# Visual-Behavior/detr-tensorflow

Hardware: AMD Instinct MI355X
Metric: images/sec training step, DETR-R50 800x1333 bs=8/GPU (higher is better)
Workload: dtype bf16

## Files before the change

### detr-tensorflow_amd/csrc/common.h

```cpp
#pragma once
#include <hip/hip_runtime.h>
#include <stdint.h>
#include <stdio.h>
#include <stdarg.h>
#include <stdlib.h>

#include "../../include/detr_hip.h"

namespace detr {

void set_error(const char *fmt, ...);

#define DETR_REQUIRE(cond, ...)                 \
    do {                                        \
        if (!(cond)) {                          \
            ::detr::set_error(__VA_ARGS__);     \
            return -1;                          \
        }                                       \
    } while (0)

#define DETR_LAUNCH_CHECK(name)                                                         \
    do {                                                                                \
        hipError_t e__ = hipGetLastError();                                             \
        if (e__ != hipSuccess) {                                                        \
// ... 32 lines not shown
    T_DGRAD_S2_CLASSES,
    T_WGRAD_FUSED,
    T_WGRAD_FUSED_WGS,
    T_WGRAD_TILE,
    T_STEM_ROWS,
    T_ATTN_WAVES,
    T_ATTN_SPLIT,
    T_GEMM_K64,
    T_EPI_WIDE,
    T_SLAB_TS,
    T_GEMM_RING,
    T_RING_NS,
    T_RING_BN,
    T_RING_WGS,
    T_RING_ROWS,
    T_RING_WTILE,
    T_CONV_DMA,
    T_SPLIT3_T128,
    T_X3_DB,
    T_X3_T192,
    T_X3_WG_ROUNDS,
    T_X3_CONV,
    T_SPLIT3_ALL,
    T_COUNT
};
int tune(TuneKey k);

static inline bool aligned16(const void *p) { return (reinterpret_cast<uintptr_t>(p) & 15) == 0; }
static inline int cdiv(long long a, long long b) { return (int)((a + b - 1) / b); }
static inline int capped_grid(long long total, int block, int cap) {
    const long long g = (total + block - 1) / block;
    return (int)(g > cap ? cap : (g < 1 ? 1 : g));
}

__host__ __device__ __forceinline__ uint32_t mix32(uint32_t x) {
    x ^= x >> 16; x *= 0x7feb352du;
    x ^= x >> 15; x *= 0x846ca68bu;
    x ^= x >> 16;
    return x;
}
__host__ __device__ __forceinline__ uint32_t drop_key(uint32_t site, const uint32_t *step) {
    return mix32((step ? *step : 0u) + site * 0x9E3779B9u);
}
__host__ __device__ __forceinline__ uint32_t drop_hash(uint32_t key, unsigned long long pair) {
    const uint32_t key2 = key * 0x85EBCA6Bu + 0xC2B2AE35u;
    uint32_t x = (uint32_t)pair ^ key;
// ... 40 lines not shown
```

### detr-tensorflow_amd/csrc/common.hip

```cpp
#include "common.h"
#include <string.h>

namespace detr {
static thread_local char g_err[512] = "";
void set_error(const char *fmt, ...) {
    va_list ap;
    va_start(ap, fmt);
    vsnprintf(g_err, sizeof(g_err), fmt, ap);
    va_end(ap);
}
static const char *const g_tune_names[T_COUNT] = {
    "DETR_HIP_GEMM_TILE",
    "DETR_HIP_SPLIT_XCD",
    "DETR_HIP_GEMM_STREAM",
    "DETR_HIP_GEMM_GROUP",
    "DETR_HIP_STREAM_SL",
    "DETR_HIP_STREAM_NW",
    "DETR_HIP_CONV_HALO",
    "DETR_HIP_CONV_TILE",
    "DETR_HIP_DGRAD_S2_CLASSES",
    "DETR_HIP_WGRAD_FUSED",
    "DETR_HIP_WGRAD_FUSED_WGS",
    "DETR_HIP_WGRAD_TILE",
    "DETR_HIP_STEM_ROWS",
    "DETR_HIP_ATTN_WAVES",
    "DETR_HIP_ATTN_SPLIT",
    "DETR_HIP_GEMM_K64",
    "DETR_HIP_EPI_WIDE",
    "DETR_HIP_SLAB_TS",
    "DETR_HIP_GEMM_RING",
    "DETR_HIP_RING_NS",
    "DETR_HIP_RING_BN",
    "DETR_HIP_RING_WGS",
    "DETR_HIP_RING_ROWS",
    "DETR_HIP_RING_WTILE",
    "DETR_HIP_CONV_DMA",
    "DETR_HIP_SPLIT3_T128",
    "DETR_HIP_X3_DB",
    "DETR_HIP_X3_T192",
    "DETR_HIP_X3_WG_ROUNDS",
    "DETR_HIP_X3_CONV",
    "DETR_HIP_SPLIT3_ALL",
};
static int g_tune[T_COUNT];
static void load_tuning() {
    for (int i = 0; i < T_COUNT; ++i) {
        const char *v = getenv(g_tune_names[i]);
        __atomic_store_n(&g_tune[i], v ? atoi(v) : 0, __ATOMIC_RELAXED);
    }
}
static const bool g_tune_loaded = (load_tuning(), true);
int tune(TuneKey k) { return __atomic_load_n(&g_tune[k], __ATOMIC_RELAXED); }
}

extern "C" int detr_hip_reload_tuning(void) {
    detr::load_tuning();
    return 0;
}
extern "C" const char *detr_hip_last_error(void) { return detr::g_err; }
extern "C" int detr_hip_abi_version(void) { return DETR_HIP_ABI_VERSION; }
__global__ __launch_bounds__(256) void zero_fill_kernel(uint4 *__restrict__ p16, size_t n16, unsigned char *__restrict__ tail, int ntail) {
    const uint4 z = make_uint4(0u, 0u, 0u, 0u);
    for (size_t i = blockIdx.x * (size_t)blockDim.x + threadIdx.x; i < n16; i += (size_t)gridDim.x * blockDim.x) p16[i] = z;
    if (blockIdx.x == 0 && (int)threadIdx.x < ntail) tail[threadIdx.x] = 0;
}
// ... 206 lines not shown
```

### detr-tensorflow_amd/csrc/gemm_f32.hip

```cpp
#include "gemm_core.h"
#include "gemm_bf16_core.h"
#include "gemm_stream.h"

#include "gemm_kernels.h"
#include "gemm_x3.h"
#include "gemm_ring.h"

namespace detr {

struct ReduceOne {
    const float *ws; int splits; long long part_stride; int rows, cols; float *C; long long ldc;
    float alpha; const float *scale; int vec; const float *rs_ws; float *rs_out; float rs_alpha; int nblocks;
    int ts_bm, ts_bn, ts_tn;
};
struct ReduceGroupArgs { ReduceOne r[GEMM_MAX_GROUP]; };

template <int G>
__device__ __forceinline__ void splitk_reduce_body(const float *__restrict__ ws, int splits, long long part_stride,
                                                   int rows, int cols, float *__restrict__ C, long long ldc,
                                                   float alpha, const float *__restrict__ scale, int vec,
                                                   const float *__restrict__ rs_ws, float *__restrict__ rs_out,
                                                   float rs_alpha, const int bid, const int nbid,
                                                   const int ts_bm = 0, const int ts_bn = 0, const int ts_tn = 1) {
    constexpr int OUT = 256 / G;
// ... 537 lines not shown
    if (!(p.bf16c && g.a16 && g.b16 && p.ak && p.batch == 1 && p.split == 1 && !g.rowsum && !d->ln_y)) return false;
    if (!(d->K % RING_BK == 0 && d->K >= 2 * RING_BK && d->N >= 128 && d->N % 8 == 0 && d->lda % 8 == 0 && d->ldb % 8 == 0 && aligned16(d->A) &&
          aligned16(d->B))) return false;
    const bool tall = d->M >= 4096 && d->K >= 512;
    const bool dec_ffn = d->M >= 512 && d->K >= 1024;
    const bool k256 = d->K == 256 && d->N >= 1024 && (d->M >= 16384 || (d->M >= 4096 && !p.bk));
    if (mode != 1 && !(tall || dec_ffn || k256)) return false;
    return gemm_ring_plan(d->M, d->N, d->K, rp);
}

static bool gemm_ring_f32_eligible(const GemmPlan &p, RingPlan &rp) {
    const detr_gemm_desc *d = p.d;
    const GemmArgs &g = p.g;
    const int mode = tune(T_GEMM_RING);
    if (mode == 2) return false;
    if (p.bf16c || p.split3 || g.a16 || g.b16 || !p.ak || p.batch != 1 || p.split != 1 || g.rowsum || d->ln_y) return false;
    if (d->c_dtype || d->r_dtype || d->m_dtype) return false;
    if (!(d->K % 32 == 0 && d->K >= 64 && d->N >= 128 && d->lda % 4 == 0 && d->ldb % 4 == 0 && aligned16(d->A) && aligned16(d->B) &&
          (p.bk || d->N % 4 == 0))) return false;
    if (mode != 1 && !(d->M >= 16384)) return false;
    return gemm_ring_f32_plan(d->M, d->N, d->K, rp);
}

static int gemm_launch(const GemmPlan &p, hipStream_t s) {
    const GemmArgs &g = p.g;
    const detr_gemm_desc *d = p.d;
    const int batch = p.batch;
    const bool ak = p.ak, bk = p.bk;
    if (d->ln_y) return gemm_ln_launch(p, s);
    {
        RingPlan rp;
        const bool ring_first = tune(T_GEMM_STREAM) != 3 && gemm_ring_eligible(p, rp);
        if (!ring_first && gemm_stream_eligible(p)) {
            gemm_stream_launch(p, s);
            DETR_LAUNCH_CHECK("gemm (stream)");
            return 0;
        }
        if (ring_first) {
            if (gemm_ring_launch(g, bk, rp, s)) return -1;
            DETR_LAUNCH_CHECK("gemm (ring)");
            if (d->defer_out) d->defer_out->splits = 0;
            return 0;
        }
        if (gemm_ring_f32_eligible(p, rp)) {
            if (gemm_ring_f32_launch(g, bk, rp, s)) return -1;
            DETR_LAUNCH_CHECK("gemm (ring, fp32)");
            if (d->defer_out) d->defer_out->splits = 0;
            return 0;
        }
    }
    const bool ring_wgrad = p.bf16c && (p.tile == 1 || p.tile == 6 || p.tile == 7) && g.a16 && g.b16 && !ak && !bk && batch == 1 && p.split > 1 &&
                            g.slab_ts && !g.rowsum && d->M % 8 == 0 && d->N % 8 == 0 && d->lda % 8 == 0 && d->ldb % 8 == 0 && aligned16(d->A) &&
                            aligned16(d->B) && tune(T_GEMM_RING) != 2 && tune(T_GEMM_RING) != 3;
    DETR_REQUIRE(ring_wgrad || (p.tile != 6 && p.tile != 7), "gemm: the 128 x 256 / 256 x 128 tiles exist for the ring weight gradient only "
                 "(tile-ordered slabs in a workspace of detr_hip_workspace_bytes_gemm bytes are required)");
    if (ring_wgrad) {
        if (gemm_ring_wgrad_launch(g, p.ts_bm, p.ts_bn, p.split, s)) return -1;
    } else if (p.bf16c) {
        if (p.tile == 2) launch_cfg_bf16<128, 64, 2, 2>(g, batch, s, ak, bk);
        else if (p.tile == 4) launch_cfg_bf16<64, 128, 2, 2>(g, batch, s, ak, bk);
        else if (p.tile == 0) launch_cfg_bf16<64, 64, 2, 2>(g, batch, s, ak, bk, p.deep);
        else launch_cfg_bf16<128, 128, 2, 2>(g, batch, s, ak, bk, p.deep);
    } else if (p.split3 && p.tile == 8) launch_x3<192, 128>(g, batch, s, ak, bk);
    else if (p.split3 && p.tile == 1) launch_x3<128, 128>(g, batch, s, ak, bk);
    else if (p.split3 && p.tile == 2) launch_x3<128, 64>(g, batch, s, ak, bk);
    else if (p.split3) launch_x3<64, 64>(g, batch, s, ak, bk);
    else if (p.tile == 1) launch_cfg<128, 128, 2, 2>(g, batch, s, ak, bk);
    else if (p.tile == 2) launch_cfg<128, 64, 2, 2>(g, batch, s, ak, bk);
    else if (p.tile == 3) launch_cfg<128, 32, 4, 1>(g, batch, s, ak, bk);
    else if (p.tile == 4) launch_cfg<64, 256, 1, 4>(g, batch, s, ak, bk);
    else if (p.tile == 5) launch_cfg<256, 64, 4, 1>(g, batch, s, ak, bk);
    else launch_cfg<64, 64, 2, 2>(g, batch, s, ak, bk);
    DETR_LAUNCH_CHECK("gemm");
    if (p.partial && d->defer_out) {
        detr_reduce_desc *o = d->defer_out;
        o->ws = d->workspace; o->splits = p.split; o->part_stride = p.part; o->rows = d->M; o->cols = d->N;
// ... 2 lines not shown
        o->rs_out = d->rowsum_a; o->rs_alpha = d->rowsum_alpha;
        o->ts_bm = p.ts_bm; o->ts_bn = p.ts_bn; o->ts_tiles_n = p.ts_tn;
        return 0;
    }
    if (d->defer_out) d->defer_out->splits = 0;
    if (p.partial) {
        launch_splitk_reduce(d->workspace, p.split, p.part, d->M, d->N, d->C, d->ldc, p.final_e.alpha, p.final_e.scale, s,
                             d->rowsum_a ? d->workspace + (long long)p.split * p.part : nullptr, d->rowsum_a, d->rowsum_alpha,
                             p.ts_bm, p.ts_bn, p.ts_tn);
        DETR_LAUNCH_CHECK("gemm split-k reduce");
    }
    return 0;
}

extern "C" int detr_hip_gemm_family(const detr_gemm_desc *d) {
    GemmPlan p;
    if (gemm_prepare(d, p)) return -1;
    if (d->ln_y) return 4;
    RingPlan rp;
    const bool ring_first = tune(T_GEMM_STREAM) != 3 && gemm_ring_eligible(p, rp);
    if (!ring_first && gemm_stream_eligible(p)) return 1;
    if (ring_first) return 2;
    if (gemm_ring_f32_eligible(p, rp)) return 3;
    const GemmArgs &g = p.g;
    const bool ring_wgrad = p.bf16c && (p.tile == 1 || p.tile == 6 || p.tile == 7) && g.a16 && g.b16 && !p.ak && !p.bk && p.batch == 1 && p.split > 1 &&
                            g.slab_ts && !g.rowsum && d->M % 8 == 0 && d->N % 8 == 0 && d->lda % 8 == 0 && d->ldb % 8 == 0 && aligned16(d->A) &&
                            aligned16(d->B) && tune(T_GEMM_RING) != 2 && tune(T_GEMM_RING) != 3;
    return ring_wgrad ? 5 : 0;
}

extern "C" int detr_hip_gemm_f32(const detr_gemm_desc *d, void *stream) {
    GemmPlan p;
    if (gemm_prepare(d, p)) return -1;
    return gemm_launch(p, (hipStream_t)stream);
}

template <bool AK, bool BKC>
static void launch_group_f32(const GemmGroupArgs &G, dim3 grid, hipStream_t s, bool split3) {
    if (split3) hipLaunchKernelGGL((gemm_x3_group_kernel<64, 64, AK, BKC>), grid, dim3(GEMM_THREADS), 0, s, G);
    else hipLaunchKernelGGL((gemm_f32_group_kernel<64, 64, 2, 2, AK, BKC>), grid, dim3(GEMM_THREADS), 0, s, G);
}
template <bool AK, bool BKC, bool A16, bool B16>
static void launch_group_bf16(const GemmGroupArgs &G, dim3 grid, hipStream_t s) {
    hipLaunchKernelGGL((gemm_bf16c_group_kernel<64, 64, 2, 2, AK, BKC, A16, B16>), grid, dim3(GEMM_THREADS), 0, s, G);
}

extern "C" int detr_hip_gemm_group_f32(const detr_gemm_desc *descs, int32_t n, void *stream) {
    DETR_REQUIRE(descs != nullptr && n >= 1 && n <= 64, "gemm group: 1..64 descriptors");
    hipStream_t s = (hipStream_t)stream;
    int done = 0;
    while (done < n) {
        const int m = (n - done) < GEMM_MAX_GROUP ? (n - done) : GEMM_MAX_GROUP;
        GemmPlan p[GEMM_MAX_GROUP];
        for (int i = 0; i < m; ++i) {
            DETR_REQUIRE(!descs[done + i].ln_y, "gemm group: the fused LayerNorm (ln_y) exists for single launches only");
            if (gemm_prepare(descs + done + i, p[i])) return -1;
        }
        bool same = m > 1 && tune(T_GEMM_GROUP) != 2;
        for (int i = 0; i < m && same; ++i)
            same = p[i].tile == 0 && p[i].batch == 1 && p[i].bf16c == p[0].bf16c && p[i].split3 == p[0].split3 && p[i].ak == p[0].ak && p[i].bk == p[0].bk &&
                   p[i].g.a16 == p[0].g.a16 && p[i].g.b16 == p[0].g.b16 && (p[i].split == 1 || p[i].partial) &&
                   !gemm_stream_eligible(p[i]);
        if (same) { RingPlan rp; for (int i = 0; i < m && same; ++i) same = !gemm_ring_eligible(p[i], rp) && !gemm_ring_f32_eligible(p[i], rp); }
        if (!same) {
            for (int i = 0; i < m; ++i)
                if (gemm_launch(p[i], s)) return -1;
            done += m;
            continue;
        }
        GemmGroupArgs G;
        G.n = m;
        G.work_off[0] = 0;
        for (int i = 0; i < m; ++i) {
            G.g[i] = p[i].g;
            G.g[i].tiles_m = cdiv(p[i].g.M, 64);
            G.g[i].tiles_n = cdiv(p[i].g.N, 64);
            G.work_off[i + 1] = G.work_off[i] + G.g[i].tiles_m * G.g[i].tiles_n * p[i].split;
        }
        for (int i = m; i < GEMM_MAX_GROUP; ++i) { G.g[i] = G.g[0]; G.work_off[i + 1] = G.work_off[m]; }
        const dim3 grid((unsigned)G.work_off[m]);
        const bool ak = p[0].ak, bk = p[0].bk, a16 = p[0].g.a16 != 0, b16 = p[0].g.b16 != 0;
#define DETR_GROUP_BF16(A16_, B16_)                                          \
    do {                                                                     \
        if (ak && bk) launch_group_bf16<true, true, A16_, B16_>(G, grid, s);    \
        else if (ak) launch_group_bf16<true, false, A16_, B16_>(G, grid, s);    \
        else if (bk) launch_group_bf16<false, true, A16_, B16_>(G, grid, s);    \
        else launch_group_bf16<false, false, A16_, B16_>(G, grid, s);           \
    } while (0)
        if (p[0].bf16c) {
            if (a16 && b16) DETR_GROUP_BF16(true, true);
            else if (a16) DETR_GROUP_BF16(true, false);
            else if (b16) DETR_GROUP_BF16(false, true);
            else DETR_GROUP_BF16(false, false);
        } else if (ak && bk) launch_group_f32<true, true>(G, grid, s, p[0].split3);
        else if (ak) launch_group_f32<true, false>(G, grid, s, p[0].split3);
        else if (bk) launch_group_f32<false, true>(G, grid, s, p[0].split3);
        else launch_group_f32<false, false>(G, grid, s, p[0].split3);
#undef DETR_GROUP_BF16
        DETR_LAUNCH_CHECK("gemm group");
        ReduceGroupArgs R;
        int nr = 0;
        unsigned rx = 1;
        bool all_small = true, any_small = false;
        for (int i = 0; i < m; ++i) {
            const detr_gemm_desc *d = p[i].d;
            if (d->defer_out) {
                detr_reduce_desc *o = d->defer_out;
                o->splits = 0;
                if (p[i].partial) {
                    o->ws = d->workspace; o->splits = p[i].split; o->part_stride = p[i].part; o->rows = d->M; o->cols = d->N;
                    o->C = d->C; o->ldc = d->ldc; o->alpha = p[i].final_e.alpha; o->scale = p[i].final_e.scale;
                    o->rs_ws = d->rowsum_a ? d->workspace + (long long)p[i].split * p[i].part : nullptr;
// ... 77 lines not shown
```

### detr-tensorflow_amd/csrc/gemm_ring.h

```cpp
#pragma once
#include "gemm_kernels.h"

namespace detr {

typedef __attribute__((address_space(3))) void lds_void_t;
constexpr int RING_BK = 64;
constexpr int RING_THREADS = 512;
constexpr int RING_STAGE_ROW = RING_BK * 2;

struct RingArgs {
    GemmArgs g;
    int tile_rows;
    int a_rows8;
    int stage_bytes;
    int dump_off;
};

struct RingPlan {
    int tm, tn, ns;
    int tile_rows, tiles_m, tiles_n, wgs;
    int a_rows8, stage_bytes, dump_off, lds_bytes;
    double cost;
};
bool gemm_ring_plan(int M, int N, int K, RingPlan &p);
int gemm_ring_wgrad_launch(const GemmArgs &g, int bm, int bn, int split, hipStream_t s);
int gemm_ring_launch(const GemmArgs &g, bool b_kcontig, const RingPlan &p, hipStream_t s);
bool gemm_ring_f32_plan(int M, int N, int K, RingPlan &p);
int gemm_ring_f32_launch(const GemmArgs &g, bool b_kcontig, const RingPlan &p, hipStream_t s);

template <int N>
__device__ __forceinline__ void ring_wait_vmcnt() {
    static_assert(N >= 0 && N < 64, "vmcnt is a 6-bit counter");
    asm volatile("s_waitcnt vmcnt(%0)" ::"n"(N) : "memory");
}

__device__ __forceinline__ void ring_dma_piece(u32x4 rs, unsigned lds_addr, unsigned voff) {
    asm volatile("s_mov_b32 m0, %0\n\ts_nop 0\n\tbuffer_load_dwordx4 %1, %2, 0 offen lds" ::"s"(lds_addr), "v"(voff), "s"(rs) : "memory", "m0");
}
__device__ __forceinline__ u32x4 ring_rsrc(const void *base, unsigned bytes) {
    const unsigned long long b = (unsigned long long)base;
    u32x4 r;
    r[0] = (unsigned)b;
    r[1] = (unsigned)(b >> 32) & 0xFFFFu;
    r[2] = bytes;
    r[3] = 0x00020000u;
    return r;
}
__device__ __forceinline__ unsigned ring_lds_addr(char *p) {
// ... 382 lines not shown
            __builtin_amdgcn_sched_barrier(0);
            cur = (cur + 1 == NS) ? 0 : cur + 1;
            nxt = (nxt + 1 == NS) ? 0 : nxt + 1;
        }
    };
    if (nmi == TM) kloop(std::integral_constant<int, TM>{});
    else if (TM >= 2 && nmi == TM - 1) kloop(std::integral_constant<int, (TM >= 2 ? TM - 1 : 0)>{});
    else if (TM >= 3 && nmi == TM - 2) kloop(std::integral_constant<int, (TM >= 3 ? TM - 2 : 0)>{});
    else if (TM >= 4 && nmi == TM - 3) kloop(std::integral_constant<int, (TM >= 4 ? TM - 3 : 0)>{});
    else kloop(std::integral_constant<int, 0>{});
    ring_wait_vmcnt<0>();
    __syncthreads();
    epilogue<BM, BN, WGM, WGN, false>(acc, reinterpret_cast<float *>(ring_smem), g.C, g.ldc, row_end, g.N, m0, n0, wm, wn, lane, wave, g.e);
}

template <int TM, int TN, bool BKC, int NS>
__global__ __launch_bounds__(RING_THREADS) void gemm_ring_f32_kernel(RingArgs ra) {
#if defined(__HIP_DEVICE_COMPILE__)
    gemm_ring_f32_body<TM, TN, BKC, NS>(ra, xcd_remap((int)blockIdx.x, (int)gridDim.x));
#endif
}

template <int TM, int TN, int NS>
__device__ __forceinline__ void gemm_ring_wgrad_body(const RingArgs &ra) {
    constexpr int BM = 64 * TM, BN = 128 * TN, WGM = 2, WGN = 4;
    static_assert(TM % 2 == 0, "the A image is made of 128-row pieces");
    using T = TileCfg<BM, BN, WGM, WGN>;
    extern __shared__ __attribute__((aligned(1024))) char ring_smem[];
    const GemmArgs &g = ra.g;
    const int tid = threadIdx.x, lane = tid & 63;
    const int wave = __builtin_amdgcn_readfirstlane(tid >> 6);
    const int wm = wave / WGN, wn = wave % WGN;
    const int tiles = g.tiles_m * g.tiles_n;
    const int id = xcd_remap((int)blockIdx.x, (int)gridDim.x);
    const int tile = id % tiles, split = id / tiles;
    const int tn = tile % g.tiles_n, tm = tile / g.tiles_n;
    const int m0 = tm * BM, n0 = tn * BN;
    const int nkt32 = (g.K + BF_BK - 1) / BF_BK;
    const int per = (nkt32 + g.split_k - 1) / g.split_k;
    const int kbeg = split * per * BF_BK;
    const int kend = min(g.K, kbeg + per * BF_BK);
    if (kbeg >= kend) return;
    RingDmaMN<BM> la;
    RingDmaMN<BN> lb;
    la.init(g.A, g.lda, m0, g.M, kend, lane, wave);
    lb.init(g.B, g.ldb, n0, g.N, kend, lane, wave);
    f32x16 acc[TM][TN];
#pragma unroll
    for (int i = 0; i < TM; ++i)
#pragma unroll
        for (int j = 0; j < TN; ++j)
#pragma unroll
            for (int r = 0; r < 16; ++r) acc[i][j][r] = 0.0f;
    constexpr int A_BYTES = BM * RING_STAGE_ROW, STAGE = (BM + BN) * RING_STAGE_ROW, PW = TM + 2 * TN;
    const unsigned lds0 = ring_lds_addr(ring_smem);
    int atr[TM], btr[TN];
#pragma unroll
// ... 15 lines not shown
        ring_stage<TM, TM, TN, false, false>(ring_smem + cur * STAGE, ring_smem + cur * STAGE + A_BYTES, acc, 0, atr, 0, btr, xo, la, lb,
                                             kbeg + (t + NS - 1) * RING_BK, kend, lds0, nxt * STAGE, nxt * STAGE + A_BYTES, 0);
        __builtin_amdgcn_sched_barrier(0);
        cur = (cur + 1 == NS) ? 0 : cur + 1;
        nxt = (nxt + 1 == NS) ? 0 : nxt + 1;
    }
    ring_wait_vmcnt<0>();
    float4 *slab = reinterpret_cast<float4 *>(g.C + (long long)split * g.part_stride + (long long)tile * (BM * BN));
    const int w2 = 2 * wm + (wn >> 1);
#pragma unroll
    for (int mi = 0; mi < TM; ++mi)
#pragma unroll
        for (int ni = 0; ni < TN; ++ni) {
            const int blk = (w2 * TM + mi) * (2 * TN) + (wn & 1) * TN + ni;
#pragma unroll
            for (int q = 0; q < 4; ++q)
                slab[(blk * 4 + q) * 64 + lane] = make_float4(acc[mi][ni][4 * q], acc[mi][ni][4 * q + 1], acc[mi][ni][4 * q + 2], acc[mi][ni][4 * q + 3]);
        }
}

template <int TM, int TN, int NS>
__global__ __launch_bounds__(RING_THREADS) void gemm_ring_wgrad_kernel(RingArgs ra) {
#if defined(__HIP_DEVICE_COMPILE__)
    gemm_ring_wgrad_body<TM, TN, NS>(ra);
#endif
}

}
```

### detr-tensorflow_amd/csrc/gemm_ring.hip

```cpp
#include "gemm_ring.h"

namespace detr {

bool gemm_ring_plan(int M, int N, int K, RingPlan &p) {
    if (M < 1 || N < 128 || K < RING_BK || K % RING_BK != 0) return false;
    const int force_bn = tune(T_RING_BN), force_wgs = tune(T_RING_WGS), force_ns = tune(T_RING_NS), force_rows = tune(T_RING_ROWS);
    int bn = 128;
    if (force_bn == 256 && N >= 256) bn = 256;
    const int tiles_n = cdiv(N, bn);
    int rows = 176, ns = 2;
    if (cdiv(M, 176) * tiles_n < 320) {
        rows = (int)(((long long)M * tiles_n + 199) / 200);
        rows = (rows + 3) & ~3;
        if (rows > 176) rows = 176;
        ns = 3;
    }
    if (force_wgs > 0) {
        const int tm_ = force_wgs / tiles_n > 0 ? force_wgs / tiles_n : 1;
        rows = (cdiv(M, tm_) + 3) & ~3;
    }
    if (force_rows >= 8) rows = (force_rows + 3) & ~3;
    if (rows < 8) rows = 8;
    if (rows > 256) return false;
    p.tile_rows = rows;
// ... 122 lines not shown
    if (!reserved) {
        hipError_t e = hipFuncSetAttribute(reinterpret_cast<const void *>(gemm_ring_wgrad_kernel<TM, TN, NS>), hipFuncAttributeMaxDynamicSharedMemorySize, 160 * 1024);
        DETR_REQUIRE(e == hipSuccess, "gemm (ring wgrad): cannot reserve LDS: %s", hipGetErrorString(e));
        reserved = true;
    }
    hipLaunchKernelGGL((gemm_ring_wgrad_kernel<TM, TN, NS>), dim3((unsigned)wgs), dim3(RING_THREADS), (size_t)LDS, s, ra);
    return 0;
}

int gemm_ring_wgrad_launch(const GemmArgs &g, int bm, int bn, int split, hipStream_t s) {
    RingArgs ra;
    ra.g = g;
    ra.g.tiles_m = cdiv(g.M, bm);
    ra.g.tiles_n = cdiv(g.N, bn);
    ra.tile_rows = ra.a_rows8 = ra.stage_bytes = ra.dump_off = 0;
    const int wgs = ra.g.tiles_m * ra.g.tiles_n * split;
    if (bm == 128 && bn == 128) return tune(T_RING_NS) == 3 ? ring_wgrad_launch_one<2, 1, 3>(ra, wgs, s) : ring_wgrad_launch_one<2, 1, 4>(ra, wgs, s);
    if (bm == 128 && bn == 256) return ring_wgrad_launch_one<2, 2, 3>(ra, wgs, s);
    if (bm == 256 && bn == 128) return ring_wgrad_launch_one<4, 1, 3>(ra, wgs, s);
    DETR_REQUIRE(false, "gemm (ring wgrad): no instantiation for %d x %d tiles", bm, bn);
    return -1;
}

}

extern "C" int detr_hip_gemm_ring_plan(int32_t M, int32_t N, int32_t K, int32_t *out) {
    detr::RingPlan p;
    if (!detr::gemm_ring_plan(M, N, K, p)) return 0;
    if (out) {
        out[0] = p.tm; out[1] = p.tn; out[2] = p.ns; out[3] = p.tile_rows; out[4] = p.tiles_m; out[5] = p.tiles_n; out[6] = p.wgs; out[7] = p.lds_bytes;
    }
    return 1;
}
```

### detr-tensorflow_amd/detr_tf/_hip.py

```python
import ctypes
import os
from ctypes import POINTER, Structure, byref, c_float, c_int32, c_int64, c_size_t, c_void_p

import torch

_HERE = os.path.dirname(os.path.abspath(__file__))
LIB_PATH = os.environ.get("DETR_HIP_LIB") or os.path.join(os.path.dirname(_HERE), "lib", "libdetr_hip.so")

f32p = c_void_p


class ReduceDesc(Structure):
    _fields_ = [("ws", c_void_p), ("splits", c_int32), ("part_stride", c_int64), ("rows", c_int32), ("cols", c_int32),
                ("C", c_void_p), ("ldc", c_int64), ("alpha", c_float), ("scale", c_void_p),
                ("rs_ws", c_void_p), ("rs_out", c_void_p), ("rs_alpha", c_float),
                ("ts_bm", c_int32), ("ts_bn", c_int32), ("ts_tiles_n", c_int32)]


class GemmDesc(Structure):
    _fields_ = [("M", c_int32), ("N", c_int32), ("K", c_int32),
                ("A", c_void_p), ("lda", c_int64), ("a_kcontig", c_int32),
                ("B", c_void_p), ("ldb", c_int64), ("b_kcontig", c_int32),
                ("C", c_void_p), ("ldc", c_int64),
                ("batch", c_int32), ("batch_inner", c_int32),
# ... 162 lines not shown
                ("t_crowd", c_void_p), ("t_area", c_void_p), ("sM_b", c_int64), ("sizes", c_void_p),
                ("thresholds", ctypes.c_double * COCO_MAX_THR), ("area_ranges", ctypes.c_double * (2 * COCO_MAX_AREA)),
                ("rec_score", c_void_p), ("rec_class", c_void_p), ("rec_rank", c_void_p), ("rec_flags", c_void_p),
                ("npig", c_void_p), ("status", c_void_p)]


class SetLossDesc(Structure):
    _fields_ = [("levels", c_int32), ("B", c_int32), ("Q", c_int32), ("C", c_int32), ("R", c_int32),
                ("logits", c_void_p), ("sL_l", c_int64), ("sL_b", c_int64), ("sL_q", c_int64),
                ("boxes", c_void_p), ("sB_l", c_int64), ("sB_b", c_int64), ("sB_q", c_int64),
                ("t_bbox", c_void_p), ("t_class", c_void_p),
                ("background_class", c_int32)]


_SIGNATURES = {
    "detr_hip_abi_version": [],
    "detr_hip_reload_tuning": [],
    "detr_hip_struct_layout": [c_int32, POINTER(c_int32), c_int32],
    "detr_hip_memset_zero": [c_void_p, c_size_t, c_void_p],
    "detr_hip_gemm_f32": [POINTER(GemmDesc), c_void_p],
    "detr_hip_gemm_group_f32": [POINTER(GemmDesc), c_int32, c_void_p],
    "detr_hip_gemm_family": [POINTER(GemmDesc)],
    "detr_hip_gemm_ring_plan": [c_int32, c_int32, c_int32, POINTER(c_int32)],
    "detr_hip_splitk_reduce_many": [POINTER(ReduceDesc), c_int32, c_void_p],
    "detr_hip_conv3x3_f32": [POINTER(Conv3x3Desc), c_int32, c_void_p],
    "detr_hip_maxpool3x3s2_fwd_bf16": [c_void_p, c_void_p, c_void_p, c_int32, c_int32, c_int32, c_int32, c_int32, c_int32, c_void_p],
    "detr_hip_maxpool3x3s2_bwd_bf16": [c_void_p, c_void_p, c_void_p, c_void_p, c_int32, c_int32, c_int32, c_int32, c_int32, c_int32,
                                       c_void_p],
    "detr_hip_cvt_bf16": [f32p, c_void_p, c_int64, c_void_p],
    "detr_hip_scale_cols_bf16": [f32p, f32p, c_void_p, c_int64, c_int32, c_void_p],
    "detr_hip_scale_cols_bf16_group": [c_void_p, c_int32, c_void_p],
    "detr_hip_stem_conv7x7_f32": [POINTER(StemDesc), c_int32, c_void_p],
    "detr_hip_maxpool3x3s2_fwd_f32": [f32p, f32p, c_void_p, c_int32, c_int32, c_int32, c_int32, c_int32, c_int32, c_void_p],
    "detr_hip_maxpool3x3s2_bwd_f32": [f32p, c_void_p, f32p, f32p, c_int32, c_int32, c_int32, c_int32, c_int32, c_int32, c_void_p],
    "detr_hip_subsample2_fwd_f32": [f32p, f32p, c_int32, c_int32, c_int32, c_int32, c_int32, c_int32, c_void_p],
    "detr_hip_subsample2_bwd_f32": [f32p, f32p, c_int32, c_int32, c_int32, c_int32, c_int32, c_int32, c_void_p],
    "detr_hip_layernorm_fwd": [POINTER(LayerNormDesc), c_void_p],
    "detr_hip_layernorm_bwd": [POINTER(LayerNormDesc), c_void_p],
    "detr_hip_attention_fwd": [POINTER(AttnDesc), c_void_p],
    "detr_hip_attention_bwd": [POINTER(AttnDesc), c_void_p],
    "detr_hip_attention_dropmask": [POINTER(AttnDesc), c_void_p],
    "detr_hip_attention_dropmask_many": [POINTER(AttnDesc), c_int32, c_void_p],
    "detr_hip_attention_fwd_masked": [POINTER(AttnDesc), c_void_p, c_void_p],
    "detr_hip_attention_bwd_masked": [POINTER(AttnDesc), c_void_p, c_void_p],
    "detr_hip_attention_weights": [POINTER(AttnDesc), c_void_p, c_void_p, c_int64, c_void_p],
    "detr_hip_padding_mask_prepare": [c_void_p, c_int32, c_int32, c_int32, c_int32, c_int32, f32p, f32p, c_void_p, f32p, c_void_p, c_void_p],
# ... 751 lines not shown
```

### detr-tensorflow_amd/detr_tf/engine.py

```python
import math
import os
from ctypes import byref, c_float

import numpy as np
import torch

from . import _hip as hip
from .params import ParamStore, RESNET50_BLOCKS, block_names, bn_conv_pairs, stem_names

D = 256
HEADS = 8
HD = 32
FF = 2048
BN_EPS = 1e-5
KERAS_BN_EPS = 1.001e-5
LN_EPS = 1e-5
DEFER_REDUCE = os.environ.get("DETR_HIP_DEFER_REDUCE", "1") != "0"
WGRAD_STREAM = os.environ.get("DETR_HIP_WGRAD_STREAM", "1") != "0"
BWD_FUSED = os.environ.get("DETR_HIP_BWD_FUSED", "1") != "0"
DROPMASK_AHEAD = int(os.environ.get("DETR_HIP_DROPMASK_AHEAD", "2") or 0)
QK_ALPHA = float(HD) ** -0.5 * 1.4426950408889634


def mix32(x):
    x &= 0xFFFFFFFF
    x ^= x >> 16
    x = (x * 0x7FEB352D) & 0xFFFFFFFF
    x ^= x >> 15
    x = (x * 0x846CA68B) & 0xFFFFFFFF
    x ^= x >> 16
    return x


def step_seed(base_seed, step_no, rank=0):
    return mix32(mix32((base_seed + 0x9E3779B9 * step_no) & 0xFFFFFFFF) ^ ((rank * 0x85EBCA6B) & 0xFFFFFFFF))


def position_embedding_sine_host(H, W, num_pos_features=128, temperature=10000.0, eps=1e-6):
    y = (np.arange(1, H + 1, dtype=np.float32) / np.float32(H + eps) * np.float32(2 * math.pi)).astype(np.float32)
    x = (np.arange(1, W + 1, dtype=np.float32) / np.float32(W + eps) * np.float32(2 * math.pi)).astype(np.float32)
    k = np.arange(num_pos_features, dtype=np.float32)
# ... 191 lines not shown
            self._fold_table = torch.tensor(rows, dtype=torch.int64).to(self.device)
            self._fold_keep = [self.bn_scale, self._bufs]
        hip.call("detr_hip_scale_cols_bf16_group", self._fold_table.data_ptr(), self._fold_table.shape[0])

    def _scaled_kernel(self, conv_name, bn_name):
        w = self.P.views[conv_name]
        co = w.shape[-1]
        if self.compute == 1 and conv_name != f"{self._stem['conv']}/kernel":
            return self.buf(f"ws16:{conv_name}", w.shape, torch.bfloat16)
        ws = self.buf(f"ws:{conv_name}", w.shape)
        if self._stale(f"ws:{conv_name}"):
            hip.call("detr_hip_scale_cols_f32", w.data_ptr(), self.bn_scale[bn_name].data_ptr(), ws.data_ptr(),
                     w.numel() // co, co)
        return ws

    def _conv1x1_fwd(self, x, M, cin, cout, conv_name, bn_name, out, residual=None, act=1, maskbits_out=None):
        ws = self._scaled_kernel(conv_name, bn_name)
        shift = self.bn_shift[bn_name]
        ldr = cout if residual is not None else 0
        hip.gemm(M, cout, cin, x, cin, 1, ws, cout, 0, out, cout, bias=shift, residual=residual, ldr=ldr, act=act,
                 maskbits_out=maskbits_out)

    @staticmethod
    def _wgrad(M_out, N_out, K_red, A, lda, Bm, ldb, C, ldc, scale=None, alpha=1.0):
        sk = hip.pick_split_k(M_out, N_out, K_red)
        if sk > 1:
            hip.gemm(M_out, N_out, K_red, A, lda, 0, Bm, ldb, 0, C, ldc, alpha=alpha, scale=scale, split_k=sk)
        else:
            hip.gemm(M_out, N_out, K_red, A, lda, 0, Bm, ldb, 0, C, ldc, alpha=alpha, scale=scale, residual=C, ldr=ldc)

    def _colsum(self, x2d, out, alpha=1.0):
        rows, cols = x2d.shape
        n = int(hip.load().detr_hip_colsum_det_scratch_floats(rows, cols))
        scratch = self.buf(f"colsum:{rows}x{cols}", (n,))
        hip.call("detr_hip_colsum_det_f32", x2d.data_ptr(), out.data_ptr(), rows, cols, x2d.stride(0), c_float(alpha),
                 scratch.data_ptr(), n)

    def _ln_fwd(self, x, pfx, y, tag, add=None, y2=None, y16=None):
        rows = x.shape[0]
        mean = self.buf(f"{tag}:mean", (rows,))
        rstd = self.buf(f"{tag}:rstd", (rows,))
        hip.layernorm_fwd(x, self.P.views[f"{pfx}/gamma"], self.P.views[f"{pfx}/beta"], y, mean, rstd, LN_EPS, add=add, y2=y2,
                          y16=y16)

    def _ln_spec(self, rows, pfx, y, tag, add=None, y2=None, y16=None, ffn=False):
        if self.compute != 1 or ffn:
            return None
        return dict(gamma=self.P.views[f"{pfx}/gamma"], beta=self.P.views[f"{pfx}/beta"], y=y, mean=self.buf(f"{tag}:mean", (rows,)),
                    rstd=self.buf(f"{tag}:rstd", (rows,)), eps=LN_EPS, add=add, y2=y2, y16=y16)

    def _side_begin(self, on):
        self._side_on = bool(on)
# ... 687 lines not shown
            fused_ok = BWD_FUSED and self.compute == 1 and adt == torch.bfloat16 and d2 == 256 and g.is_cuda
            fuse3, fuse_down = fused_ok and d1 == 64, False
            if m["first"] and not (tfb and strided):
                idg = self.buf(f"scratch:idg:{cin}:{h}", (B, h, w, cin), adt)

                fuse_down = fused_ok and not strided and cin == 64

                def dg_down(g=g, idg=idg):
                    if strided:
                        dxs = self.buf(f"scratch:dxs:{cin}:{ho}", (B, ho, wo, cin), adt)
                        hip.gemm(M_out, cin, d2, g, d2, 1, wsd, d2, 1, dxs, cin)
                        hip.call("detr_hip_subsample2_bwd_f32", dxs.data_ptr(), idg.data_ptr(), B, h, w, cin // f32c, ho, wo)
                    elif fuse_down:
                        hip.conv1x1_bwd_fused(g.view(M_out, d2), xs.view(M_out, cin), wsd.view(cin, d2), idg.view(M_out, cin), G[f"{n['down']}/kernel"].view(cin, d2),
                                              self.buf(f"bwdfused:slabs:down:{M_out}", (hip.conv1x1_bwd_fused_scratch_floats(M_out),)),
                                              scale=self.bn_scale[n["bnd"]], use_mask=False)
                    else:
                        hip.gemm(M_out, cin, d2, g, d2, 1, wsd, d2, 1, idg, cin)
                on_side(dg_down)
                if ws_on:
                    idg_ready = torch.cuda.Event()
                    idg_ready.record(wside)

            def wg3(g=g, fuse3=fuse3, fuse_down=fuse_down):
                if not fuse3:
                    self._wgrad(d1, d2, M_out, y2, d1, g, d2, G[f"{n['conv3']}/kernel"], d2, scale=self.bn_scale[n["bn3"]])
                bias_grad(n["conv3"], n["bn3"], g, M_out, d2)
                if m["first"]:
                    if not fuse_down:
                        self._wgrad(cin, d2, M_out, xs, cin, g, d2, G[f"{n['down']}/kernel"], d2, scale=self.bn_scale[n["bnd"]])
                    bias_grad(n["down"], n["bnd"], g, M_out, d2)
            on_side(wg3)
            dz2 = self.buf(f"scratch:dz2:{d1}:{ho}{par}", (B, ho, wo, d1), adt)
            if fuse3:
                hip.conv1x1_bwd_fused(g.view(M_out, d2), y2.view(M_out, d1), ws3.view(d1, d2), dz2.view(M_out, d1), G[f"{n['conv3']}/kernel"].view(d1, d2),
                                      self.buf(f"bwdfused:slabs:{M_out}", (hip.conv1x1_bwd_fused_scratch_floats(M_out),)),
                                      scale=self.bn_scale[n["bn3"]], use_mask=True)
            else:
                hip.gemm(M_out, d1, d2, g, d2, 1, ws3, d2, 1, dz2, d1, mask=y2, ldmask=d1)

            def wg2():
                hip.conv3x3(2, y1, dz2, G[f"{n['conv2']}/kernel"], B, h1, w1, d1, ho, wo, d1, s2, scale=self.bn_scale[n["bn2"]],
                            pad=m["dil"], dilation=m["dil"])
                bias_grad(n["conv2"], n["bn2"], dz2, M_out, d1)
            on_side(wg2)
            dz1 = self.buf(f"scratch:dz1:{d1}:{h1}{par}", (B, h1, w1, d1), adt)
            hip.conv3x3(1, dz2, ws2, dz1, B, h1, w1, d1, ho, wo, d1, s2, mask=y1, pad=m["dil"], dilation=m["dil"])

            def wg1():
                self._wgrad(cin, d1, M1, x1, cin, dz1, d1, G[f"{n['conv1']}/kernel"], d1, scale=self.bn_scale[n["bn1"]])
                bias_grad(n["conv1"], n["bn1"], dz1, M1, d1)
            on_side(wg1)
            side_mark(bi)
            side_wait(bi + 1)
            is_first_block = bi == 0
            gx = self.buf(f"scratch:gx:{cin}:{h}:{bi & 1}", (B, h, w, cin), adt)
            mask = None if is_first_block else x
            xbits = None if is_first_block else self._block_meta[bi - 1].get("out_bits")
            if tfb and strided:
                dxs = self.buf(f"scratch:dxs:{cin}:{ho}", (B, ho, wo, cin), adt)
                hip.gemm(M_out, cin, d2, g, d2, 1, wsd, d2, 1, dxs, cin)
                hip.gemm(M_out, cin, d1, dz1, d1, 1, ws1, d1, 1, dxs, cin, residual=dxs, ldr=cin,
                         mask=(None if is_first_block else xs), ldmask=(0 if is_first_block else cin))
                hip.call("detr_hip_subsample2_bwd_f32", dxs.data_ptr(), gx.data_ptr(), B, h, w, cin // f32c, ho, wo)
            else:
                if idg_ready is not None:
                    main.wait_event(idg_ready)
                if xbits is not None:
                    hip.gemm(M_in, cin, d1, dz1, d1, 1, ws1, d1, 1, gx, cin, residual=idg, ldr=cin, mask=xbits, ldmask=xbits.stride(0))
                else:
                    hip.gemm(M_in, cin, d1, dz1, d1, 1, ws1, d1, 1, gx, cin, residual=idg, ldr=cin, mask=mask,
                             ldmask=(cin if mask is not None else 0))
            g = gx
# ... 21 lines not shown
```

### include/detr_hip.h

```cpp
#ifndef DETR_HIP_H
#define DETR_HIP_H

#include <stddef.h>
#include <stdint.h>

#ifdef __cplusplus
extern "C" {
#endif

#define DETR_HIP_ABI_VERSION 9

const char *detr_hip_last_error(void);
int detr_hip_abi_version(void);
int detr_hip_reload_tuning(void);
int detr_hip_struct_layout(int32_t which, int32_t *out, int32_t cap);
int detr_hip_memset_zero(void *ptr, size_t bytes, void *stream);

typedef struct detr_reduce_desc {
    const float *ws; int32_t splits; int64_t part_stride; int32_t rows, cols;
    float *C; int64_t ldc; float alpha; const float *scale;
    const float *rs_ws; float *rs_out; float rs_alpha;
    int32_t ts_bm, ts_bn, ts_tiles_n;
} detr_reduce_desc;

// ... 261 lines not shown
int detr_hip_clip_adam_f32(float *param, const float *g, float *m, float *v, const int32_t *chunk_tensor,
                           const int64_t *chunk_start, const int64_t *seg_end, const int32_t *tensor_group,
                           const float *sumsq, const float *hyper, int32_t n_chunks, int32_t chunk,
                           void *stream);
int detr_hip_set_floats8_f32(float *dst, float v0, float v1, float v2, float v3, float v4, float v5, float v6,
                             float v7, void *stream);
int detr_hip_axpy_f32(float *acc, const float *g, float a, int64_t n, void *stream);

int detr_hip_set_floats16_f32(float *dst, const float *values, void *stream);
int detr_hip_global_clip_scale_f32(const float *sumsq, const int32_t *chunk_tensor, const int32_t *tensor_group,
                                   const float *hyper, int32_t n_chunks, float *scale, void *stream);
int detr_hip_adamw_f32(float *param, const float *g, float *m, float *v, const int32_t *chunk_tensor,
                       const int64_t *chunk_start, const int64_t *seg_end, const int32_t *tensor_group,
                       const float *sumsq, const float *hyper, const float *scale, int32_t n_chunks, int32_t chunk,
                       void *stream);

int64_t detr_hip_workspace_bytes_gemm(const detr_gemm_desc *d);
int64_t detr_hip_workspace_bytes_conv3x3(const detr_conv3x3_desc *d, int32_t mode);
int64_t detr_hip_workspace_bytes_stem(const detr_stem_desc *d, int32_t mode);
int64_t detr_hip_workspace_bytes_layernorm(const detr_layernorm_desc *d);

int detr_hip_gemm_ring_plan(int32_t M, int32_t N, int32_t K, int32_t *out);

typedef struct {
    int32_t N, Hi, Wi, Ci, Ho, Wo, Co, stride, pad;
    const float *x;
    const float *w;
    float *y;
    float alpha;
    const float *scale;
    const float *bias;
    const float *residual;
    const float *mask;
    int32_t act;
    int32_t split;
    float *workspace; int64_t workspace_bytes;
    int32_t compute;
    int32_t w_dtype;
    int32_t x_dtype, y_dtype, r_dtype, m_dtype;
    uint8_t *maskbits_out;
    int32_t dilation;
} detr_conv3x3d_desc;
int detr_hip_conv3x3_dilated(const detr_conv3x3d_desc *d, int32_t mode, void *stream);
int64_t detr_hip_workspace_bytes_conv3x3_dilated(const detr_conv3x3d_desc *d, int32_t mode);

typedef struct {
// ... 150 lines not shown
```

Baseline: 521.0.

## Batch ring split-K weight-gradient GEMMs into a single grouped kernel launch

Adds a grouped variant of the ring split-K weight-gradient kernel. Several eligible wgrad GEMMs are packed into one launch through a work-offset table, and each workgroup finds its member by scanning the offsets. In the ResNet backward, the conv3 and downsample weight gradients are now collected and issued as a single group (optionally merged later with conv1 behind an env flag). The aim is to cut launch overhead and fill the GPU better with small wgrad GEMMs, at the cost of fixing the tile at 128x128 and choosing the stage count heuristically.

Measured after the change: 520.4. Within noise of the previous version (-0.1%).

```diff
diff --git a/detr-tensorflow_amd/csrc/common.h b/detr-tensorflow_amd/csrc/common.h
--- a/detr-tensorflow_amd/csrc/common.h
+++ b/detr-tensorflow_amd/csrc/common.h
@@ -78,6 +78,7 @@
     T_X3_WG_ROUNDS,
     T_X3_CONV,
     T_SPLIT3_ALL,
+    T_RING_GROUP,
     T_COUNT
 };
 int tune(TuneKey k);
diff --git a/detr-tensorflow_amd/csrc/common.hip b/detr-tensorflow_amd/csrc/common.hip
--- a/detr-tensorflow_amd/csrc/common.hip
+++ b/detr-tensorflow_amd/csrc/common.hip
@@ -41,6 +41,7 @@
     "DETR_HIP_X3_WG_ROUNDS",
     "DETR_HIP_X3_CONV",
     "DETR_HIP_SPLIT3_ALL",
+    "DETR_HIP_RING_GROUP",
 };
 static int g_tune[T_COUNT];
 static void load_tuning() {
diff --git a/detr-tensorflow_amd/csrc/gemm_f32.hip b/detr-tensorflow_amd/csrc/gemm_f32.hip
--- a/detr-tensorflow_amd/csrc/gemm_f32.hip
+++ b/detr-tensorflow_amd/csrc/gemm_f32.hip
@@ -583,6 +583,14 @@
     return gemm_ring_f32_plan(d->M, d->N, d->K, rp);
 }
 
+static bool gemm_ring_wgrad_eligible(const GemmPlan &p) {
+    const detr_gemm_desc *d = p.d;
+    const GemmArgs &g = p.g;
+    return p.bf16c && (p.tile == 1 || p.tile == 6 || p.tile == 7) && g.a16 && g.b16 && !p.ak && !p.bk && p.batch == 1 && p.split > 1 &&
+           g.slab_ts && !g.rowsum && d->M % 8 == 0 && d->N % 8 == 0 && d->lda % 8 == 0 && d->ldb % 8 == 0 && aligned16(d->A) &&
+           aligned16(d->B) && tune(T_GEMM_RING) != 2 && tune(T_GEMM_RING) != 3;
+}
+
 static int gemm_launch(const GemmPlan &p, hipStream_t s) {
     const GemmArgs &g = p.g;
     const detr_gemm_desc *d = p.d;
@@ -610,9 +618,7 @@
             return 0;
         }
     }
-    const bool ring_wgrad = p.bf16c && (p.tile == 1 || p.tile == 6 || p.tile == 7) && g.a16 && g.b16 && !ak && !bk && batch == 1 && p.split > 1 &&
-                            g.slab_ts && !g.rowsum && d->M % 8 == 0 && d->N % 8 == 0 && d->lda % 8 == 0 && d->ldb % 8 == 0 && aligned16(d->A) &&
-                            aligned16(d->B) && tune(T_GEMM_RING) != 2 && tune(T_GEMM_RING) != 3;
+    const bool ring_wgrad = gemm_ring_wgrad_eligible(p);
     DETR_REQUIRE(ring_wgrad || (p.tile != 6 && p.tile != 7), "gemm: the 128 x 256 / 256 x 128 tiles exist for the ring weight gradient only "
                  "(tile-ordered slabs in a workspace of detr_hip_workspace_bytes_gemm bytes are required)");
     if (ring_wgrad) {
@@ -661,11 +667,28 @@
     if (!ring_first && gemm_stream_eligible(p)) return 1;
     if (ring_first) return 2;
     if (gemm_ring_f32_eligible(p, rp)) return 3;
-    const GemmArgs &g = p.g;
-    const bool ring_wgrad = p.bf16c && (p.tile == 1 || p.tile == 6 || p.tile == 7) && g.a16 && g.b16 && !p.ak && !p.bk && p.batch == 1 && p.split > 1 &&
-                            g.slab_ts && !g.rowsum && d->M % 8 == 0 && d->N % 8 == 0 && d->lda % 8 == 0 && d->ldb % 8 == 0 && aligned16(d->A) &&
-                            aligned16(d->B) && tune(T_GEMM_RING) != 2 && tune(T_GEMM_RING) != 3;
-    return ring_wgrad ? 5 : 0;
+    return gemm_ring_wgrad_eligible(p) ? 5 : 0;
+}
+
+extern "C" int detr_hip_gemm_ring_wgrad_group_plan(int32_t n, const int32_t *M, const int32_t *N, const int32_t *K, const int32_t *split_k, int32_t *out) {
+    if (n < 1 || n > GEMM_MAX_GROUP || !M || !N || !K || !split_k) return -1;
+    GemmGroupArgs G;
+    int split[GEMM_MAX_GROUP];
+    G.n = n;
+    for (int i = 0; i < n; ++i) {
+        if (M[i] <= 0 || N[i] <= 0 || K[i] <= 0) return -1;
+        detr_gemm_desc d = {};
+        d.M = M[i]; d.N = N[i]; d.K = K[i]; d.split_k = split_k[i]; d.compute = 1;
+        split[i] = gemm_effective_split(&d);
+        G.g[i].M = M[i]; G.g[i].N = N[i];
+    }
+    const int grid = gemm_ring_wgrad_group_table(G, split);
+    if (out)
+        for (int i = 0; i < n; ++i) {
+            out[4 * i] = G.work_off[i]; out[4 * i + 1] = G.work_off[i + 1] - G.work_off[i];
+            out[4 * i + 2] = G.g[i].tiles_m * G.g[i].tiles_n; out[4 * i + 3] = split[i];
+        }
+    return grid;
 }
 
 extern "C" int detr_hip_gemm_f32(const detr_gemm_desc *d, void *stream) {
@@ -701,7 +724,9 @@
                    p[i].g.a16 == p[0].g.a16 && p[i].g.b16 == p[0].g.b16 && (p[i].split == 1 || p[i].partial) &&
                    !gemm_stream_eligible(p[i]);
         if (same) { RingPlan rp; for (int i = 0; i < m && same; ++i) same = !gemm_ring_eligible(p[i], rp) && !gemm_ring_f32_eligible(p[i], rp); }
-        if (!same) {
+        bool ring_group = !same && tune(T_RING_GROUP) != 2 && (m > 1 || tune(T_RING_GROUP) == 1);
+        for (int i = 0; i < m && ring_group; ++i) ring_group = gemm_ring_wgrad_eligible(p[i]) && p[i].tile == 1 && p[i].partial;
+        if (!same && !ring_group) {
             for (int i = 0; i < m; ++i)
                 if (gemm_launch(p[i], s)) return -1;
             done += m;
@@ -726,7 +751,12 @@
         else if (bk) launch_group_bf16<false, true, A16_, B16_>(G, grid, s);    \
         else launch_group_bf16<false, false, A16_, B16_>(G, grid, s);           \
     } while (0)
-        if (p[0].bf16c) {
+        if (ring_group) {
+            int split[GEMM_MAX_GROUP];
+            for (int i = 0; i < m; ++i) split[i] = p[i].split;
+            gemm_ring_wgrad_group_table(G, split);
+            if (gemm_ring_wgrad_group_launch(G, s)) return -1;
+        } else if (p[0].bf16c) {
             if (a16 && b16) DETR_GROUP_BF16(true, true);
             else if (a16) DETR_GROUP_BF16(true, false);
             else if (b16) DETR_GROUP_BF16(false, true);
diff --git a/detr-tensorflow_amd/csrc/gemm_ring.h b/detr-tensorflow_amd/csrc/gemm_ring.h
--- a/detr-tensorflow_amd/csrc/gemm_ring.h
+++ b/detr-tensorflow_amd/csrc/gemm_ring.h
@@ -24,6 +24,8 @@
 };
 bool gemm_ring_plan(int M, int N, int K, RingPlan &p);
 int gemm_ring_wgrad_launch(const GemmArgs &g, int bm, int bn, int split, hipStream_t s);
+int gemm_ring_wgrad_group_table(GemmGroupArgs &G, const int *split);
+int gemm_ring_wgrad_group_launch(const GemmGroupArgs &G, hipStream_t s);
 int gemm_ring_launch(const GemmArgs &g, bool b_kcontig, const RingPlan &p, hipStream_t s);
 bool gemm_ring_f32_plan(int M, int N, int K, RingPlan &p);
 int gemm_ring_f32_launch(const GemmArgs &g, bool b_kcontig, const RingPlan &p, hipStream_t s);
@@ -452,17 +454,15 @@
 }
 
 template <int TM, int TN, int NS>
-__device__ __forceinline__ void gemm_ring_wgrad_body(const RingArgs &ra) {
+__device__ __forceinline__ void gemm_ring_wgrad_body(const GemmArgs &g, const int id) {
     constexpr int BM = 64 * TM, BN = 128 * TN, WGM = 2, WGN = 4;
     static_assert(TM % 2 == 0, "the A image is made of 128-row pieces");
     using T = TileCfg<BM, BN, WGM, WGN>;
     extern __shared__ __attribute__((aligned(1024))) char ring_smem[];
-    const GemmArgs &g = ra.g;
     const int tid = threadIdx.x, lane = tid & 63;
     const int wave = __builtin_amdgcn_readfirstlane(tid >> 6);
     const int wm = wave / WGN, wn = wave % WGN;
     const int tiles = g.tiles_m * g.tiles_n;
-    const int id = xcd_remap((int)blockIdx.x, (int)gridDim.x);
     const int tile = id % tiles, split = id / tiles;
     const int tn = tile % g.tiles_n, tm = tile / g.tiles_n;
     const int m0 = tm * BM, n0 = tn * BN;
@@ -524,8 +524,22 @@
 template <int TM, int TN, int NS>
 __global__ __launch_bounds__(RING_THREADS) void gemm_ring_wgrad_kernel(RingArgs ra) {
 #if defined(__HIP_DEVICE_COMPILE__)
-    gemm_ring_wgrad_body<TM, TN, NS>(ra);
+    gemm_ring_wgrad_body<TM, TN, NS>(ra.g, xcd_remap((int)blockIdx.x, (int)gridDim.x));
 #endif
 }
 
-}
+template <int TM, int TN, int NS>
+__global__ __launch_bounds__(RING_THREADS) void gemm_ring_wgrad_group_kernel(GemmGroupArgs G) {
+#if defined(__HIP_DEVICE_COMPILE__)
+    const int b = (int)blockIdx.x;
+    if (b >= G.work_off[G.n]) return;
+    int m = 0;
+#pragma unroll
+    for (int i = 1; i < GEMM_MAX_GROUP; ++i)
+        if (i < G.n && b >= G.work_off[i]) m = i;
+    const int first = G.work_off[m];
+    gemm_ring_wgrad_body<TM, TN, NS>(G.g[m], xcd_remap(b - first, G.work_off[m + 1] - first));
+#endif
+}
+
+}
diff --git a/detr-tensorflow_amd/csrc/gemm_ring.hip b/detr-tensorflow_amd/csrc/gemm_ring.hip
--- a/detr-tensorflow_amd/csrc/gemm_ring.hip
+++ b/detr-tensorflow_amd/csrc/gemm_ring.hip
@@ -168,6 +168,39 @@
     return -1;
 }
 
+int gemm_ring_wgrad_group_table(GemmGroupArgs &G, const int *split) {
+    G.work_off[0] = 0;
+    for (int i = 0; i < GEMM_MAX_GROUP; ++i) {
+        int wgs = 0;
+        if (i < G.n) {
+            G.g[i].tiles_m = cdiv(G.g[i].M, 128);
+            G.g[i].tiles_n = cdiv(G.g[i].N, 128);
+            wgs = G.g[i].tiles_m * G.g[i].tiles_n * split[i];
+        }
+        G.work_off[i + 1] = G.work_off[i] + wgs;
+    }
+    return G.work_off[G.n];
+}
+
+template <int NS>
+static int ring_wgrad_group_launch_one(const GemmGroupArgs &G, hipStream_t s) {
+    constexpr int LDS = NS * (128 + 128) * RING_STAGE_ROW;
+    static bool reserved = false;
+    if (!reserved) {
+        hipError_t e = hipFuncSetAttribute(reinterpret_cast<const void *>(gemm_ring_wgrad_group_kernel<2, 1, NS>), hipFuncAttributeMaxDynamicSharedMemorySize, LDS);
+        DETR_REQUIRE(e == hipSuccess, "gemm (ring wgrad group): cannot reserve LDS: %s", hipGetErrorString(e));
+        reserved = true;
+    }
+    hipLaunchKernelGGL((gemm_ring_wgrad_group_kernel<2, 1, NS>), dim3((unsigned)G.work_off[G.n]), dim3(RING_THREADS), (size_t)LDS, s, G);
+    return 0;
+}
+int gemm_ring_wgrad_group_launch(const GemmGroupArgs &G, hipStream_t s) {
+    DETR_REQUIRE(G.n >= 1 && G.n <= GEMM_MAX_GROUP && G.work_off[G.n] > 0, "gemm (ring wgrad group): 1..%d members", GEMM_MAX_GROUP);
+    const int force = tune(T_RING_NS), fg = tune(T_RING_GROUP);
+    const bool two = force == 2 || fg == 3 || (force != 3 && fg != 4 && G.work_off[G.n] <= 2 * 256);
+    return two ? ring_wgrad_group_launch_one<2>(G, s) : ring_wgrad_group_launch_one<3>(G, s);
+}
+
 }
 
 extern "C" int detr_hip_gemm_ring_plan(int32_t M, int32_t N, int32_t K, int32_t *out) {
diff --git a/detr-tensorflow_amd/detr_tf/_hip.py b/detr-tensorflow_amd/detr_tf/_hip.py
--- a/detr-tensorflow_amd/detr_tf/_hip.py
+++ b/detr-tensorflow_amd/detr_tf/_hip.py
@@ -208,6 +208,7 @@
     "detr_hip_gemm_group_f32": [POINTER(GemmDesc), c_int32, c_void_p],
     "detr_hip_gemm_family": [POINTER(GemmDesc)],
     "detr_hip_gemm_ring_plan": [c_int32, c_int32, c_int32, POINTER(c_int32)],
+    "detr_hip_gemm_ring_wgrad_group_plan": [c_int32, POINTER(c_int32), POINTER(c_int32), POINTER(c_int32), POINTER(c_int32), POINTER(c_int32)],
     "detr_hip_splitk_reduce_many": [POINTER(ReduceDesc), c_int32, c_void_p],
     "detr_hip_conv3x3_f32": [POINTER(Conv3x3Desc), c_int32, c_void_p],
     "detr_hip_maxpool3x3s2_fwd_bf16": [c_void_p, c_void_p, c_void_p, c_int32, c_int32, c_int32, c_int32, c_int32, c_int32, c_void_p],
diff --git a/detr-tensorflow_amd/detr_tf/engine.py b/detr-tensorflow_amd/detr_tf/engine.py
--- a/detr-tensorflow_amd/detr_tf/engine.py
+++ b/detr-tensorflow_amd/detr_tf/engine.py
@@ -17,6 +17,7 @@
 LN_EPS = 1e-5
 DEFER_REDUCE = os.environ.get("DETR_HIP_DEFER_REDUCE", "1") != "0"
 WGRAD_STREAM = os.environ.get("DETR_HIP_WGRAD_STREAM", "1") != "0"
+WGRAD_GROUP_LATE = os.environ.get("DETR_HIP_WGRAD_GROUP_LATE", "0") == "1"
 BWD_FUSED = os.environ.get("DETR_HIP_BWD_FUSED", "1") != "0"
 DROPMASK_AHEAD = int(os.environ.get("DETR_HIP_DROPMASK_AHEAD", "2") or 0)
 QK_ALPHA = float(HD) ** -0.5 * 1.4426950408889634
@@ -254,12 +255,23 @@
                  maskbits_out=maskbits_out)
 
     @staticmethod
-    def _wgrad(M_out, N_out, K_red, A, lda, Bm, ldb, C, ldc, scale=None, alpha=1.0):
+    def _wgrad_call(M_out, N_out, K_red, A, lda, Bm, ldb, C, ldc, scale=None, alpha=1.0):
         sk = hip.pick_split_k(M_out, N_out, K_red)
+        args = (M_out, N_out, K_red, A, lda, 0, Bm, ldb, 0, C, ldc)
         if sk > 1:
-            hip.gemm(M_out, N_out, K_red, A, lda, 0, Bm, ldb, 0, C, ldc, alpha=alpha, scale=scale, split_k=sk)
+            return args, dict(alpha=alpha, scale=scale, split_k=sk)
+        return args, dict(alpha=alpha, scale=scale, residual=C, ldr=ldc)
+
+    @staticmethod
+    def _issue(calls):
+        if len(calls) == 1:
+            hip.gemm(*calls[0][0], **calls[0][1])
         else:
-            hip.gemm(M_out, N_out, K_red, A, lda, 0, Bm, ldb, 0, C, ldc, alpha=alpha, scale=scale, residual=C, ldr=ldc)
+            hip.gemm_group(calls)
+
+    @classmethod
+    def _wgrad(cls, *a, **kw):
+        cls._issue([cls._wgrad_call(*a, **kw)])
 
     def _colsum(self, x2d, out, alpha=1.0):
         rows, cols = x2d.shape
@@ -993,13 +1005,17 @@
                     idg_ready = torch.cuda.Event()
                     idg_ready.record(wside)
 
-            def wg3(g=g, fuse3=fuse3, fuse_down=fuse_down):
-                if not fuse3:
-                    self._wgrad(d1, d2, M_out, y2, d1, g, d2, G[f"{n['conv3']}/kernel"], d2, scale=self.bn_scale[n["bn3"]])
+            wg3_calls = []
+            if not fuse3:
+                wg3_calls.append(self._wgrad_call(d1, d2, M_out, y2, d1, g, d2, G[f"{n['conv3']}/kernel"], d2, scale=self.bn_scale[n["bn3"]]))
+            if m["first"] and not fuse_down:
+                wg3_calls.append(self._wgrad_call(cin, d2, M_out, xs, cin, g, d2, G[f"{n['down']}/kernel"], d2, scale=self.bn_scale[n["bnd"]]))
+
+            def wg3(g=g, calls=wg3_calls):
+                if calls and not WGRAD_GROUP_LATE:
+                    self._issue(calls)
                 bias_grad(n["conv3"], n["bn3"], g, M_out, d2)
                 if m["first"]:
-                    if not fuse_down:
-                        self._wgrad(cin, d2, M_out, xs, cin, g, d2, G[f"{n['down']}/kernel"], d2, scale=self.bn_scale[n["bnd"]])
                     bias_grad(n["down"], n["bnd"], g, M_out, d2)
             on_side(wg3)
             dz2 = self.buf(f"scratch:dz2:{d1}:{ho}{par}", (B, ho, wo, d1), adt)
@@ -1018,8 +1034,8 @@
             dz1 = self.buf(f"scratch:dz1:{d1}:{h1}{par}", (B, h1, w1, d1), adt)
             hip.conv3x3(1, dz2, ws2, dz1, B, h1, w1, d1, ho, wo, d1, s2, mask=y1, pad=m["dil"], dilation=m["dil"])
 
-            def wg1():
-                self._wgrad(cin, d1, M1, x1, cin, dz1, d1, G[f"{n['conv1']}/kernel"], d1, scale=self.bn_scale[n["bn1"]])
+            def wg1(late=wg3_calls if WGRAD_GROUP_LATE else []):
+                self._issue(late + [self._wgrad_call(cin, d1, M1, x1, cin, dz1, d1, G[f"{n['conv1']}/kernel"], d1, scale=self.bn_scale[n["bn1"]])])
                 bias_grad(n["conv1"], n["bn1"], dz1, M1, d1)
             on_side(wg1)
             side_mark(bi)
diff --git a/include/detr_hip.h b/include/detr_hip.h
--- a/include/detr_hip.h
+++ b/include/detr_hip.h
@@ -307,6 +307,8 @@
 
 int detr_hip_gemm_ring_plan(int32_t M, int32_t N, int32_t K, int32_t *out);
 
+int detr_hip_gemm_ring_wgrad_group_plan(int32_t n, const int32_t *M, const int32_t *N, const int32_t *K, const int32_t *split_k, int32_t *out);
+
 typedef struct {
     int32_t N, Hi, Wi, Ci, Ho, Wo, Co, stride, pad;
     const float *x;
```
